# AnnaLew/pangenomix

Hardware: AMD Instinct MI355X
Metric: proteins/sec clustered at 0.8 identity + pan/core iters/sec, 400-genome set (higher is better)
Workload: dtype i32

## Files before the change

pangenomix_amd/csrc/cluster.hip:

```cpp
#include <algorithm>
#include <chrono>
#include <cstdlib>
#include <cmath>
#include <type_traits>
#include <functional>
#include <condition_variable>
#include <mutex>
#include <thread>
#include <vector>

#include "cluster_layout.h"
#include "cluster_tables.h"
#include "pgx_internal.h"

namespace {

using namespace pgxc;

constexpr uint32_t kWindowMax = 65536;
constexpr int kDiscoveryRounds = 2;
constexpr uint32_t kBlockCap = 4096;
constexpr uint32_t kBlockCapMin = 64;

constexpr uint32_t kMaxLen = 1u << 22;
// ... 1084 lines not shown
        FT_LAP(ft, 9);
    }
    flush_pairs();
#ifdef PGX_FTIME
    FT_LAP(ft, 10);
    if (lane == 0 && NEWONLY && !A.qlist) {
        for (int i = 0; i < 12; ++i) atomicAdd(&g_ftime[i], ft.acc[i]);
        atomicAdd(&g_ftime[12], 1ull);
    }
#endif
    if (lane == 0 && wave_visits) atomicAdd(&s_visits, wave_visits);
    __syncthreads();
    if (threadIdx.x == 0 && s_visits) atomicAdd(A.visits, s_visits);
}

__global__ __launch_bounds__(256) void index_strike_kernel(DevSeqs S, const uint32_t *__restrict__ list, uint32_t n,
                                                          IndexLine *__restrict__ lines, uint32_t *__restrict__ pool) {
    const uint32_t lane = threadIdx.x & 63u, rmask = entry_rmask(S);
    for (uint32_t w = blockIdx.x * 4 + (threadIdx.x >> 6); w < n; w += gridDim.x * 4) {
        const uint32_t k = list[w];
        const uint64_t o = S.off[k];
        const uint32_t nw = S.wcnt[k];
        for (uint32_t i = lane; i < nw; i += 64) {
            IndexLine &L = lines[S.wcode[o + i]];
            const uint32_t hi = L.len;
            for (uint32_t j = line_len_prev(L); j < hi; ++j) {
                uint32_t *e = j < kInline ? &L.e[j] : &pool[L.ovf + 1u + (j - kInline)];
                if ((*e & rmask) == k) { *e = rmask; break; }
            }
        }
    }
}

enum { C_NW = 0, C_NK = 1, C_EVAL0 = 2, C_BLK = 3, C_OPEN = 4, C_NEW = 5, C_SEG0 = 6, C_TOUCH = 7, C_ERR = 8, C_ROUND_OPEN = 9, C_ZERO = 10, C_WIDE = 11, C_ROUND_OPEN2 = 12, C_COUNT = 16 };
constexpr int kSelThreads = 1024;
__global__ __launch_bounds__(kSelThreads) void select_block_kernel(const unsigned long long *__restrict__ best,
                                                                  uint8_t *__restrict__ done,
                                                                  uint8_t *__restrict__ inblk, uint32_t b0,
                                                                  uint32_t nb, uint32_t block_cap,
                                                                  uint32_t *__restrict__ blk_list,
                                                                  uint32_t *__restrict__ counters,
                                                                  uint32_t *__restrict__ n_k,
                                                                  uint8_t *__restrict__ hascand_accepted,
                                                                  uint32_t window_cap, uint32_t *__restrict__ base_counters) {
    constexpr uint32_t kTiles = kWindowMax / kSelThreads;
    __shared__ uint32_t s_pre[kTiles][16];
    __shared__ uint32_t s_tile[kTiles + 1];
    const uint32_t tid = threadIdx.x, lane = tid & 63u, wave = tid >> 6;
    for (uint32_t i = tid; i < 2 * window_cap / 8; i += kSelThreads) reinterpret_cast<unsigned long long *>(hascand_accepted)[i] = 0ull;
    if (tid == 0) { *n_k = 0u; base_counters[C_TOUCH] = 0u; base_counters[C_EVAL0] = base_counters[C_NW]; }
    const uint32_t n_tiles = (nb + kSelThreads - 1) / kSelThreads;
    unsigned long long open = 0ull;
#pragma unroll 8
    for (uint32_t j = 0; j < n_tiles; ++j) {
        const uint32_t q = j * kSelThreads + tid;
        if (q >= nb) continue;
        const uint8_t ib = inblk[q];
        uint8_t d = done[q];
        const unsigned long long b = best[q];
        if (ib) { done[q] = 1; inblk[q] = 0; d = 1; }
        if (!d && b == kNoBest) open |= 1ull << j;
    }
    for (uint32_t j = 0; j < n_tiles; ++j) {
        const unsigned long long bal = __ballot((open >> j) & 1ull);
        if (lane == 0) s_pre[j][wave] = (uint32_t)__popcll(bal);
    }
    __syncthreads();
    {
        const uint32_t j = tid >> 4, w = tid & 15u;
        const uint32_t c = j < n_tiles ? s_pre[j][w] : 0u;
        uint32_t incl = c;
        for (int dd = 1; dd < 16; dd <<= 1) { const uint32_t y = __shfl_up(incl, dd, 16); if ((int)w >= dd) incl += y; }
        __syncthreads();
        if (j < n_tiles) s_pre[j][w] = incl - c;
        if (w == 15u) s_tile[j] = incl;
    }
    __syncthreads();
    if (wave == 0) {
        const uint32_t c = lane < n_tiles ? s_tile[lane] : 0u;
        uint32_t incl = c;
        for (int dd = 1; dd < 64; dd <<= 1) { const uint32_t y = __shfl_up(incl, dd); if ((int)lane >= dd) incl += y; }
        s_tile[lane] = incl - c;
        if (lane == 63u) { s_tile[kTiles] = incl; counters[0] = incl < block_cap ? incl : block_cap; counters[1] = incl; }
    }
    __syncthreads();
    for (uint32_t j = 0; j < n_tiles; ++j) {
        const bool is_open = (open >> j) & 1ull;
        const unsigned long long bal = __ballot(is_open);
        if (!is_open) continue;
        const uint32_t rank = s_tile[j] + s_pre[j][wave] + (uint32_t)__popcll(bal & ((1ull << lane) - 1ull));
        if (rank < block_cap) { const uint32_t q = j * kSelThreads + tid; blk_list[rank] = b0 + q; inblk[q] = 1; }
    }
}

__global__ __launch_bounds__(256) void list_open_kernel(const unsigned long long *__restrict__ best,
                                                       const uint8_t *__restrict__ done, uint32_t b0, uint32_t nb,
                                                       uint32_t *__restrict__ ulist, uint32_t *__restrict__ c,
                                                       uint32_t which) {
    const uint32_t q = blockIdx.x * blockDim.x + threadIdx.x;
    if (q == 0) {
        c[C_EVAL0] = c[C_NW]; c[C_SEG0] = c[C_NEW]; c[C_TOUCH] = 0u;
        c[which ? C_ROUND_OPEN : C_ROUND_OPEN2] = 0u;
    }
    if (q >= nb) return;
    if (!done[q] && best[q] == kNoBest) ulist[atomicAdd(&c[which ? C_ROUND_OPEN2 : C_ROUND_OPEN], 1u)] = b0 + q;
}
constexpr uint32_t kMaxChunks = 32;
struct Chunks { uint32_t n; uint32_t begin[kMaxChunks + 1]; };
__device__ __forceinline__ uint32_t chunk_of(const Chunks &C, uint32_t ql) {
    uint32_t c = 0;
    for (uint32_t t = 1; t < C.n; ++t) c += ql >= C.begin[t];
    return c;
}
__global__ __launch_bounds__(256) void first_open_kernel(DevSeqs S, const uint32_t *__restrict__ ulist,
                                                        const uint32_t *__restrict__ n_open, uint32_t b0,
                                                        uint32_t epoch, uint32_t *__restrict__ first, uint32_t stride,
                                                        Chunks C, const int32_t *__restrict__ req_aan,
                                                        uint8_t *__restrict__ decided) {
    const uint32_t lane = threadIdx.x & 63u, n = *n_open;
    for (uint32_t w = blockIdx.x * 4 + (threadIdx.x >> 6); w < n; w += gridDim.x * 4) {
        const uint32_t k = ulist[w], ql = k - b0, c = chunk_of(C, ql);
        const uint64_t o = S.off[k];
        const uint32_t nw = S.wcnt[k], tag = (epoch << 16) | (65535u - ql);
        uint32_t sum = 0;
        for (uint32_t i = lane; i < nw; i += 64) {
            uint32_t *slot = first + (size_t)S.wcode[o + i] * stride + c;
            const uint32_t v = *slot;
            if (v < tag) atomicMax(slot, tag);
            else if (v > tag && (v >> 16) == epoch) sum += S.wmult[o + i];
        }
        for (int d = 32; d > 0; d >>= 1) sum += __shfl_xor(sum, d);
        if (lane == 0) decided[ql] = sum != 0u && (int32_t)sum >= req_aan[k];
    }
}
__global__ __launch_bounds__(256) void certain_kernel(DevSeqs S, const uint32_t *__restrict__ ulist,
                                                     const uint32_t *__restrict__ n_open, uint32_t b0,
                                                     uint32_t both, uint32_t epoch,
                                                     const uint32_t *__restrict__ first, uint32_t stride, Chunks C,
                                                     const int32_t *__restrict__ req_aan,
                                                     const uint8_t *__restrict__ decided,
                                                     uint8_t *__restrict__ done, uint32_t *__restrict__ list,
                                                     uint32_t *__restrict__ n_list) {
    __shared__ uint32_t s_cnt[4][kMaxChunks];
    const uint32_t lane = threadIdx.x & 63u, n = *n_open;
    uint32_t *cnt = s_cnt[threadIdx.x >> 6];
    for (uint32_t w = blockIdx.x * 4 + (threadIdx.x >> 6); w < n; w += gridDim.x * 4) {
        const uint32_t k = ulist[w], ql = k - b0;
        if (decided[ql]) continue;
        const uint32_t c = chunk_of(C, ql);
        const int32_t t0 = req_aan[k];
        bool cand = false;
        for (uint32_t strand = 0; strand < (both ? 2u : 1u) && !cand; ++strand) {
            const uint32_t ks = strand ? S.n_fwd + k : k;
            const uint64_t o = S.off[ks];
            const uint32_t nw = S.wcnt[ks];
            if (lane < kMaxChunks) cnt[lane] = 0u;
            __builtin_amdgcn_fence(__ATOMIC_RELEASE, "workgroup");
            __builtin_amdgcn_wave_barrier();
            uint32_t sum = 0;
            for (uint32_t i = lane; i < nw; i += 64) {
                const uint32_t m = S.wmult[o + i];
                const uint32_t *rec = first + (size_t)S.wcode[o + i] * stride;
                for (uint32_t t4 = 0; t4 <= c; t4 += 4) {
                    uint32_t v[4];
                    if (stride >= 4) { const uint4 x = *reinterpret_cast<const uint4 *>(rec + t4); v[0] = x.x; v[1] = x.y; v[2] = x.z; v[3] = x.w; }
                    else { v[0] = rec[0]; v[1] = stride > 1 ? rec[1] : 0u; v[2] = 0u; v[3] = 0u; }
#pragma unroll
                    for (uint32_t j = 0; j < 4; ++j) {
                        const uint32_t t = t4 + j;
                        if (t > c || (v[j] >> 16) != epoch) continue;
                        if (t < c) atomicAdd(&cnt[t], m);
                        else if (65535u - (v[j] & 65535u) < ql) sum += m;
                    }
                }
            }
            for (int d = 32; d > 0; d >>= 1) sum += __shfl_xor(sum, d);
            __builtin_amdgcn_fence(__ATOMIC_RELEASE, "workgroup");
            __builtin_amdgcn_wave_barrier();
            __builtin_amdgcn_fence(__ATOMIC_ACQUIRE, "workgroup");
            uint32_t mx = lane < c ? cnt[lane] : 0u;
            mx = mx > sum ? mx : sum;
            for (int d = 32; d > 0; d >>= 1) { const uint32_t v = __shfl_xor(mx, d); mx = v > mx ? v : mx; }
            cand = mx != 0u && (int32_t)mx >= t0;
            __builtin_amdgcn_wave_barrier();
        }
        if (!cand && lane == 0) {
            done[ql] = 1;
            list[atomicAdd(n_list, 1u)] = k;
        }
    }
}

__global__ __launch_bounds__(256) void thresholds_kernel(const uint32_t *__restrict__ len, uint32_t n,
                                                        const int32_t *__restrict__ tab, uint32_t n_len,
                                                        int32_t *__restrict__ aa1, int32_t *__restrict__ aas,
                                                        int32_t *__restrict__ aan) {
    const uint32_t k = blockIdx.x * blockDim.x + threadIdx.x;
    if (k >= n) return;
    const uint32_t L = len[k];
    aa1[k] = tab[L]; aas[k] = tab[n_len + L]; aan[k] = tab[2 * n_len + L];
}


__global__ void retire_block_kernel(uint8_t *__restrict__ done, uint8_t *__restrict__ inblk, uint32_t nb, uint32_t final_,
                                    uint32_t *__restrict__ begin) {
    const uint32_t q = blockIdx.x * blockDim.x + threadIdx.x;
    if (q == 0 && begin) { begin[C_TOUCH] = 0u; begin[C_NK] = 0u; begin[C_EVAL0] = begin[C_NW]; }
    if (q < nb && inblk[q]) { done[q] = (uint8_t)final_; inblk[q] = 0; }
}
__global__ __launch_bounds__(256) void window_init_kernel(uint32_t *__restrict__ counters,
                                                         unsigned long long *__restrict__ best,
                                                         unsigned long long *__restrict__ rc_visits,
                                                         uint8_t *__restrict__ flags, uint32_t window_cap) {
    const uint32_t q = blockIdx.x * blockDim.x + threadIdx.x;
    if (q < C_COUNT && q != C_ERR) counters[q] = 0u;
    if (q >= window_cap) return;
    best[q] = kNoBest;
    if (rc_visits) rc_visits[q] = 0ull;
    if (q < 4 * window_cap / 8) reinterpret_cast<unsigned long long *>(flags)[q] = 0ull;
// ... 843 lines not shown
            if (out_strand) out_strand[i] = 0;
        }
    });
    if (n_in == 0) { if (stats) *stats = S; return PGX_OK; }

    DevBuf d_res, d_off, d_len, d_wcode, d_wmult, d_wcnt, d_aa1, d_aas, d_aan, d_lines, d_pool[2], d_idx,
        d_newbits, d_touched, d_first, d_best_own, d_rcvis, d_counters, d_visits, d_pairsW, d_pairsK, d_blk_list,
        d_ulist, d_new_list, d_flags, d_gscratch, d_order, d_list, d_gather, d_pk, d_pkoff,
        d_counters2, d_best2, d_flags2, d_pairsW2, d_gscratch2,
        d_thr, d_hugewords, d_xsend, d_xrecv,
        d_hist, d_sortcnt, d_tilesum, d_runs;
    {
        DevBuf *all[] = {&d_res, &d_off, &d_len, &d_wcode, &d_wmult, &d_wcnt, &d_aa1, &d_aas, &d_aan, &d_lines,
                         &d_pool[0], &d_pool[1], &d_idx, &d_newbits, &d_touched, &d_first, &d_best_own, &d_rcvis,
                         &d_counters, &d_visits, &d_pairsW, &d_pairsK, &d_blk_list, &d_ulist, &d_new_list, &d_flags,
                         &d_gscratch, &d_order, &d_list, &d_gather, &d_pk, &d_pkoff,
                         &d_counters2, &d_best2, &d_flags2, &d_pairsW2, &d_gscratch2, &d_thr, &d_hugewords,
                         &d_xsend, &d_xrecv, &d_hist, &d_sortcnt, &d_tilesum, &d_runs};
        int sl = 1;
        for (DevBuf *b : all) { b->ctx = ctx; b->slot = sl++; }
    }
    uint32_t n_codes = 1;
    for (int t = 0; t < P->word_len; ++t) n_codes *= nt ? 4u : (uint32_t)kNAA1;
    static_assert(kSegs == 4, "eight codes per word of the round's map");
    const uint32_t bm_words = (n_codes / 8 + 2 + 3) & ~3u;
    const bool overlap = !nt && !std::getenv("PGX_NO_OVERLAP");
    DevBuf d_in_len;
    d_in_len.ctx = ctx; d_in_len.slot = 0;
    PGX_HIP(d_in_len.alloc((size_t)n_in * 4));
    constexpr uint32_t kHistWords = H_BINS + kDevSortMaxLen + 1;
    PGX_HIP(d_hist.alloc((size_t)kHistWords * 4));
    PGX_HIP(d_idx.alloc(16));
    PGX_HIP(d_newbits.alloc(2 * (size_t)bm_words * 4 + 16));
    PGX_HIP(d_counters.alloc(C_COUNT * 4));
    PGX_HIP(d_visits.alloc(8));
    if (overlap) PGX_HIP(d_counters2.alloc(C_COUNT * 4));
    {
        ClearArgs ca{};
        auto seg = [&](DevBuf &b, size_t words) { ca.p[ca.n] = b.as<uint32_t>(); ca.words[ca.n] = (uint32_t)words; ++ca.n; };
        seg(d_hist, kHistWords);
        seg(d_newbits, 2 * (size_t)bm_words);
        seg(d_counters, C_COUNT);
        seg(d_visits, 2);
        if (overlap) seg(d_counters2, C_COUNT);
        ca.one = d_idx.as<uint32_t>();
        clear_kernel<<<1024, 256, 0, st>>>(ca);
        LAUNCH_CHECK();
    }
    {
        ProfScope prof(ctx, "seq_len_kernel", st);
        seq_len_kernel<<<(n_in + 3) / 4, 256, 0, st>>>(d_residues, d_offsets, n_in, total_in, d_in_len.as<uint32_t>());
        len_hist_kernel<<<std::min(64u, (n_in + 1023u) / 1024u), 1024, 0, st>>>(d_in_len.as<uint32_t>(), n_in, P->min_length,
                                                                               d_hist.as<uint32_t>());
    }
    LAUNCH_CHECK();
    HostVec<uint32_t> h_hist(ctx, 6, kHistWords);
    PGX_REQUIRE(h_hist.ok(), "out of host memory");
    PGX_HIP(hipMemcpyAsync(h_hist.data(), d_hist.p, (size_t)(H_BINS + kHistLds) * 4, hipMemcpyDeviceToHost, st));
    PGX_HIP(hipStreamSynchronize(st));
    const bool dev_sort = h_hist[H_OVER] == 0 && !std::getenv("PGX_HOST_PROLOGUE");
    uint32_t max_len = h_hist[H_MAX];
    if (dev_sort && max_len >= kHistLds) {
        PGX_HIP(hipMemcpyAsync(h_hist.data() + H_BINS + kHistLds, d_hist.as<uint32_t>() + H_BINS + kHistLds,
                               (size_t)(max_len + 1 - kHistLds) * 4, hipMemcpyDeviceToHost, st));
        PGX_HIP(hipStreamSynchronize(st));
    }
    phase("  seq_len + histogram + copy");
    const uint32_t *len_hist = h_hist.data() + H_BINS;
    uint32_t n = 0;
// ... 109 lines not shown
        uint64_t in_chunk = 0;
        uint32_t q = 0;
        for (; b0 + q < limit && q < window_cap; ++q) {
            const uint64_t w = h_len[b0 + q];
            if (chunking && in_chunk && in_chunk + w > chunk_words) {
                if (C.n == kMaxChunks) break;
                C.begin[C.n++] = q;
                in_chunk = 0;
            }
            in_chunk += w;
        }
        C.begin[C.n] = q;
        return q;
    };
    const bool need_gscratch = (uint64_t)max_len * 2 > kDiagLdsSmall;
    const uint32_t packed_len = nt ? kPackedLenNt : kPackedLenAa;
    const uint32_t gs_cells = (max_len + 64u) & ~63u;
    const uint32_t gs_stride = (max_len > packed_len ? 5u : 3u) * gs_cells;
    const uint32_t diag_grid = (uint32_t)std::max<uint64_t>(64, std::min<uint64_t>(8192, (4ull << 30) / ((uint64_t)gs_stride * 4)));
    const uint32_t align_grid = 1024;

    PGX_HIP(d_res.alloc(total + 16));
    PGX_HIP(d_off.alloc(((size_t)nv + 1) * 8));
    PGX_HIP(d_len.alloc((size_t)nv * 4));
    PGX_HIP(d_wcode.alloc((total + 16) * 4));
    PGX_HIP(d_wmult.alloc((total + 16) * 2));
    PGX_HIP(d_wcnt.alloc((size_t)nv * 4));
    PGX_HIP(d_pk.alloc(((size_t)total_pk + 16) * 4));
    PGX_HIP(d_pkoff.alloc(((size_t)nv + 1) * 4));
    PGX_HIP(d_aa1.alloc((size_t)n * 4));
    PGX_HIP(d_aas.alloc((size_t)n * 4));
    PGX_HIP(d_aan.alloc((size_t)n * 4));
    PGX_HIP(d_lines.alloc((size_t)n_codes * sizeof(IndexLine)));
    PGX_HIP(hipMemsetAsync(d_lines.p, 0, (size_t)n_codes * sizeof(IndexLine), st));
    PGX_HIP(d_best_own.alloc((size_t)window_cap * 8));
    PGX_HIP(d_rcvis.alloc((size_t)window_cap * 8));
    PGX_HIP(d_blk_list.alloc((size_t)kBlockCap * 4));
    PGX_HIP(d_ulist.alloc((size_t)window_cap * 4));
    PGX_HIP(d_new_list.alloc((size_t)window_cap * 4));
    PGX_HIP(d_flags.alloc(4 * (size_t)window_cap));
    PGX_HIP(d_list.alloc((size_t)pair_cap_k * 4));
    PGX_HIP(d_gather.alloc((size_t)pair_cap_k * sizeof(Pair)));
    PGX_HIP(d_pairsW.alloc((size_t)pair_cap * sizeof(Pair)));
    PGX_HIP(d_pairsK.alloc((size_t)pair_cap_k * sizeof(Pair)));
    if (need_gscratch) PGX_HIP(d_gscratch.alloc((size_t)diag_grid * gs_stride * 4));
    if (overlap) {
        if (!exchanging) PGX_HIP(d_best2.alloc((size_t)window_cap * 8));
        PGX_HIP(d_flags2.alloc(4 * (size_t)window_cap));
        PGX_HIP(d_pairsW2.alloc((size_t)pair_cap * sizeof(Pair)));
        if (need_gscratch) PGX_HIP(d_gscratch2.alloc((size_t)diag_grid * gs_stride * 4));
    }
    int pool_cur = 0;
    uint64_t pool_cap = 0;
    auto ensure_pool = [&](uint64_t entries, hipStream_t on) -> int {
        const uint64_t need = 8 * entries + 4096;
        if (need <= pool_cap) return PGX_OK;
        if (need > 0xFFFFFFF0ull) { pgx_set_error("pgx_cluster_greedy: word index too large for 32-bit pool offsets"); return PGX_ERR_CAPACITY; }
        const uint64_t want = std::min<uint64_t>(0xFFFFFFF0ull, need + need / 2);
        DevBuf &nb_ = d_pool[pool_cur ^ 1];
        PGX_HIP(nb_.alloc(want * 4));
        if (pool_cap) PGX_HIP(hipMemcpyAsync(nb_.p, d_pool[pool_cur].p, pool_cap * 4, hipMemcpyDeviceToDevice, on));
        pool_cur ^= 1;
        pool_cap = want;
        return PGX_OK;
    };
    PGX_HIP(d_order.alloc((size_t)n * 4));
    if (dev_sort) {
        uint32_t per = kSortShare;
        while ((uint64_t)((n_in + per - 1) / per) * n_runs > kSortCells) per *= 2;
        const uint32_t n_shares = (n_in + per - 1) / per, cells = n_shares * n_runs, tiles = (cells + kScanTile - 1) / kScanTile;
        PGX_HIP(d_sortcnt.alloc((size_t)cells * 4));
        PGX_HIP(d_tilesum.alloc((size_t)tiles * 4));
        uint32_t *const cnt = d_sortcnt.as<uint32_t>(), *const in_len = d_in_len.as<uint32_t>();
        ProfScope prof(ctx, "length_sort_kernels", st);
        ClearArgs ca{};
        ca.p[0] = cnt; ca.words[0] = cells; ca.n = 1;
        clear_kernel<<<std::min(2048u, (cells + 255u) / 256u), 256, 0, st>>>(ca);
        sort_count_kernel<<<(n_in + 255) / 256, 256, 0, st>>>(in_len, n_in, P->min_length, max_len, per, n_shares, cnt);
        tile_sum_kernel<<<tiles, 256, 0, st>>>(cnt, cells, d_tilesum.as<uint32_t>());
        tile_scan_kernel<<<tiles, 256, 0, st>>>(cnt, cells, d_tilesum.as<uint32_t>());
        sort_place_kernel<<<(n_shares + 3) / 4, 256, 0, st>>>(in_len, n_in, P->min_length, max_len, per, n_shares, cnt, n,
                                                              d_order.as<uint32_t>());
        LAUNCH_CHECK();
        PGX_HIP(hipMemcpyAsync(order.data(), d_order.p, (size_t)n * 4, hipMemcpyDeviceToHost, st));
    } else {
        PGX_HIP(hipMemcpyAsync(d_order.p, order.data(), (size_t)n * 4, hipMemcpyHostToDevice, st));
    }
    {
        const size_t runs_bytes = 2 * ((size_t)n_runs + 1) * 8;
        PGX_HIP(d_runs.alloc(runs_bytes));
        PGX_HIP(hipMemcpyAsync(d_runs.p, h_runs.data(), runs_bytes, hipMemcpyHostToDevice, st));
        const uint64_t *const dr_off = d_runs.as<uint64_t>();
        const uint32_t *const dr_pos = reinterpret_cast<const uint32_t *>(dr_off + n_runs + 1), *const dr_pk = dr_pos + n_runs + 1;
        layout_kernel<<<nv / 256 + 1, 256, 0, st>>>(dr_off, dr_pos, dr_pk, n_runs, max_len, n, nv, d_len.as<uint32_t>(),
                                                    d_off.as<uint64_t>(), d_pkoff.as<uint32_t>());
        LAUNCH_CHECK();
    }
    {
        ProfScope prof(ctx, "encode_gather_kernel", st);
        encode_gather_kernel<<<(n + 3) / 4, 256, 0, st>>>(d_residues, d_offsets, d_order.as<uint32_t>(),
                                                          d_off.as<uint64_t>(), d_res.as<uint8_t>(), n, nt ? 1 : 0);
        if (both)
            revcomp_kernel<<<(n + 3) / 4, 256, 0, st>>>(d_res.as<uint8_t>(), d_off.as<uint64_t>(),
                                                        d_len.as<uint32_t>(), n);
        pack5_kernel<<<(nv + 3) / 4, 256, 0, st>>>(d_res.as<uint8_t>(), d_off.as<uint64_t>(), d_len.as<uint32_t>(),
                                                   d_pkoff.as<uint32_t>(), nv, d_pk.as<uint32_t>());
    }
    LAUNCH_CHECK();
    {
        PGX_HIP(d_thr.alloc(3 * ((size_t)max_len + 1) * 4));
        PGX_HIP(hipMemcpyAsync(d_thr.p, h_thr.data(), 3 * ((size_t)max_len + 1) * 4, hipMemcpyHostToDevice, st));
        thresholds_kernel<<<(n + 255) / 256, 256, 0, st>>>(d_len.as<uint32_t>(), n, d_thr.as<int32_t>(), max_len + 1,
                                                          d_aa1.as<int32_t>(), d_aas.as<int32_t>(), d_aan.as<int32_t>());
        LAUNCH_CHECK();
    }
    phase("alloc + sort + layout + encode (enq)");
    {
// ... 9 lines not shown
            const uint32_t o = half * n;
            if (k32) {
                uint32_t slots = 65536;
                while (slots < 2u * max_len) slots *= 2;
                const uint32_t per_launch = std::min(k32, std::max(1u, (uint32_t)((256ull << 20) / ((uint64_t)slots * 8))));
                PGX_HIP(d_hugewords.alloc((size_t)per_launch * slots * 8));
                ProfScope prof(ctx, "words_kernel", st);
                for (uint32_t a = 0; a < k32; a += per_launch)
                    words_huge_kernel<<<std::min(per_launch, k32 - a), 1024, 0, st>>>(r8, o64, l32, o + a, o + std::min(k32, a + per_launch), wl, base,
                                                                                       nt, d_hugewords.as<uint32_t>(), slots, wc, wm, wn,
                                                                                       d_counters.as<uint32_t>() + C_ERR);
                LAUNCH_CHECK();
            }
            if ((rc = launch_words<32768, 1024>(ctx, st, r8, o64, l32, o + k32, o + k8, wl, base, nt, wc, wm, wn))) return rc;
            if ((rc = launch_words<8192, 1024>(ctx, st, r8, o64, l32, o + k8, o + k2, wl, base, nt, wc, wm, wn))) return rc;
            if ((rc = launch_words_hash<2048, 256>(ctx, st, r8, o64, l32, o + k2, o + k1k, wl, base, nt, wc, wm, wn))) return rc;
            if (k5 > k1k) {
                ProfScope prof(ctx, "words_kernel", st);
                words_wave_kernel<2048><<<(k5 - k1k + 3) / 4, 256, 0, st>>>(r8, o64, l32, o + k1k, o + k5, wl, base, nt, wc, wm, wn);
                LAUNCH_CHECK();
            }
            if (n > k5) {
                ProfScope prof(ctx, "words_kernel", st);
                words_wave_kernel<1024><<<(n - k5 + 3) / 4, 256, 0, st>>>(r8, o64, l32, o + k5, o + n, wl, base, nt, wc, wm, wn);
                LAUNCH_CHECK();
            }
        }
    }
    DevSeqs DS{d_res.as<uint8_t>(), d_off.as<uint64_t>(), d_len.as<uint32_t>(),
               d_wcode.as<uint32_t>(), d_wmult.as<uint16_t>(), d_wcnt.as<uint32_t>(),
               d_pk.as<uint32_t>(), d_pkoff.as<uint32_t>(), n, nt ? 4 : kNAA1, nt ? 4 : 2, nt ? 1 : 0, mshift};
    HostVec<uint32_t> h_wcnt(ctx, 8, n);
    PGX_REQUIRE(h_wcnt.ok(), "out of host memory");
    PGX_HIP(hipMemcpyAsync(h_wcnt.data(), d_wcnt.p, (size_t)n * 4, hipMemcpyDeviceToHost, st));

    phase("word lists (enqueue)");
    fill_host_layout();
    phase("host lengths + offsets");
    uint64_t max_window_words = 0;
    uint32_t max_chunks = 1;
    {
        Chunks C;
        size_t nf = 0;
        for (uint32_t b0 = 0, nbw; b0 < n; b0 += nbw) {
            while (nf < flush_at.size() && flush_at[nf] <= b0) ++nf;
            nbw = form_window(b0, C, nf < flush_at.size() ? flush_at[nf] : n);
            max_window_words = std::max<uint64_t>(max_window_words, h_off[b0 + nbw] - h_off[b0]);
            max_chunks = std::max(max_chunks, C.n);
        }
        if (!flush_at.empty())
            max_window_words = std::max<uint64_t>(max_window_words, h_off[std::min(n, window_cap)]);
    }
    if (chunking && flush_at.empty())
        max_window_words = std::max<uint64_t>(max_window_words,
            std::min<uint64_t>(h_off[std::min(n, window_cap)], (uint64_t)kMaxChunks * std::max<uint64_t>(chunk_words, max_len)));
    PGX_REQUIRE(max_window_words < 0xFFFFFFF0ull, "window too large");
    PGX_HIP(d_touched.alloc((max_window_words + 16) * sizeof(Deferred)));
    if (chunking && n > window_cap / 2) max_chunks = kMaxChunks;
    uint32_t tag_stride = 1;
    while (tag_stride < max_chunks) tag_stride *= 2;
    PGX_HIP(d_first.alloc((size_t)tag_stride * n_codes * 4 + 16));
    std::vector<uint32_t> rep_seq;
    HostVec<int32_t> cluster_of(ctx, 9, n, -1);
    HostVec<int32_t> iden_of(ctx, 10, n, -1);
    PGX_REQUIRE(cluster_of.ok() && iden_of.ok(), "out of host memory");
    Pinned<Pair> hW, hK;
    Pinned<unsigned long long> h_best, h_rcvis;
// ... 41 lines not shown
    uint8_t *const d_flags_set[2] = {d_flags.as<uint8_t>(), d_flags2.as<uint8_t>()};
    std::vector<uint8_t> status(window_cap);
    HostVec<uint8_t> strand_of(ctx, 11, n, (uint8_t)0);
    PGX_REQUIRE(strand_of.ok(), "out of host memory");
    std::vector<unsigned long long> winner_key(window_cap);
    std::vector<uint32_t> new_reps, order_k, rank_of(window_cap), bucket_k(kBlockCap + 2), fill_k(kBlockCap + 2), flight;
    auto real = [&](uint32_t k) { return k >= n ? k - n : k; };
    auto pair_key = [&](const Pair &pp) {
        return ((unsigned long long)(pp.q >= n) << 63) | ((unsigned long long)pp.minc << 32) | pp.r;
    };
    uint64_t n_rounds = 0;

    uint64_t gpu_pairs = 0, gpu_aligned = 0, gpu_aligned_bytes = 0, filter_walk_words = 0;
    auto account = [&](const Pair *pp, uint32_t cnt) {
        for (uint32_t i = 0; i < cnt; ++i) {
            ++gpu_pairs;
            if ((pp[i].flags & (F_DIAG_PASS | F_BAND_OK)) != (F_DIAG_PASS | F_BAND_OK)) continue;
            ++gpu_aligned;
            gpu_aligned_bytes += h_len[pp[i].q] + h_len[pp[i].r];
        }
    };
    auto window_error = [&](uint32_t e, uint32_t at) {
        pgx_set_error("pgx_cluster_greedy: capacity failure in the window at %u%s:%s%s%s%s%s%s", at,
                      exchanging ? " (on this or another process)" : "",
                      e & E_TOUCHED ? " append scratch list full;" : "", e & E_POOL ? " overflow pool of the word index full;" : "",
                      e & E_TABLE ? " exact table of the filter overflowed;" : "",
                      e & E_BAND ? " alignment band wider than 64 diagonals;" : "", e & E_PAIRS ? " candidate pair buffer overflow;" : "",
                      e & E_WORDMULT ? " a word occurs more than 65535 times in one sequence;" : "");
    };
    const bool trace = std::getenv("PGX_TRACE") != nullptr;
    const uint32_t filter_grid = 4096u;
    uint32_t epoch_idx = 0;
    uint32_t epoch_tag = 0;
    PGX_HIP(hipMemsetAsync(d_first.p, 0, (size_t)tag_stride * n_codes * 4, st));
    phase("window set-up");
    const auto t_loop0 = std::chrono::steady_clock::now();
    double t_resolve = 0.0, t_close = 0.0;
    uint64_t n_blocks = 0;
    g_wait_s = 0.0;
    std::function<int()> deferred;
    std::vector<uint32_t> members;
    uint64_t pending_words = 0;
    Chunks chunks;
    Pinned<uint8_t> h_taken;
    h_taken.bind(ctx, 14);
    if (!flush_at.empty()) { PGX_HIP(h_taken.reserve(n)); std::fill(h_taken.p, h_taken.p + n, (uint8_t)0); }
    auto drain = [&]() -> int {
        if (deferred) { int rc = deferred(); deferred = nullptr; if (rc) return rc; }
        PGX_HIP(hipStreamSynchronize(st_main));
        PGX_HIP(hipStreamSynchronize(ctx->stream2));
        return PGX_OK;
    };
    size_t next_flush = 0;
    bool sweeping = false;
    uint32_t sweep_at = 0;
    for (uint32_t cursor = 0, nb = 0; cursor < n;) {
        if (!sweeping && next_flush < flush_at.size() && cursor == flush_at[next_flush]) {
            ++next_flush;
            sweeping = true; sweep_at = cursor;
            int rc = drain(); if (rc) return rc;
        }
        const bool sweep = sweeping;
        const uint32_t b0 = sweep ? sweep_at : cursor;
        nb = form_window(b0, chunks, sweep || next_flush >= flush_at.size() ? n : flush_at[next_flush]);
        const int set = overlap ? (int)(S.sweeps & 1u) : 0;
        const hipStream_t st = set ? ctx->stream2 : st_main;
        uint32_t *const dc = dc_set[set];
// ... 130 lines not shown
                                                     dc + C_TOUCH, (uint32_t)max_window_words, dc + C_ERR);
            index_grow_kernel<<<256, 256, 0, st>>>(d_lines.as<IndexLine>(), d_poolp, d_idx.as<uint32_t>(),
                                                   (uint32_t)pool_cap, d_touched.as<Deferred>(), dc + C_TOUCH,
                                                   (uint32_t)max_window_words, dc + C_ERR);
            index_place_kernel<<<256, 256, 0, st>>>(d_lines.as<IndexLine>(), d_poolp, d_touched.as<Deferred>(),
                                                    dc + C_TOUCH, (uint32_t)max_window_words, reinterpret_cast<uint4 *>(next_map),
                                                    bm_words / 4);
            LAUNCH_CHECK();
            return PGX_OK;
        };
        auto filter_new_and_evaluate = [&](const uint32_t *d_lo, const uint32_t *d_hi) -> int {
            FilterArgs F = FA;
            F.epoch = epoch_idx; F.d_round_lo = d_lo; F.d_round_hi = d_hi;
            F.newbits = d_newbits.as<uint32_t>() + (size_t)(epoch_idx & 1u) * bm_words;
            {
                ProfScope prof(ctx, "filter_kernel<new>", st);
                auto kern = nt ? filter_kernel<true, true> : filter_kernel<false, true>;
                kern<<<std::min(filter_grid, (ns + 3) / 4), 256, 0, st>>>(DS, F);
            }
            LAUNCH_CHECK();
            filter_walk_words += window_words * (both ? 2 : 1) / shard_count;
            return evaluate_round();
        };
        uint32_t n_listed = 0;
        if (sweep) { int rc = begin_host_side(); if (rc) return rc; }
        if (!sweep) {
        if (overlap && S.sweeps > 1)
            PGX_HIP(hipStreamWaitEvent(st, ev.post[set ^ 1], 0));
        static const int n_disc = std::getenv("PGX_ROUNDS") ? std::atoi(std::getenv("PGX_ROUNDS")) : kDiscoveryRounds;
        for (int round = 0; round < n_disc; ++round) {
            if (++epoch_tag == 0xFFFFu) { PGX_HIP(hipMemsetAsync(d_first.p, 0, (size_t)tag_stride * n_codes * 4, st)); epoch_tag = 1; }
            const uint32_t which = (uint32_t)round & 1u;
            uint32_t *const d_n_open = dc + (which ? C_ROUND_OPEN2 : C_ROUND_OPEN);
            list_open_kernel<<<(nb + 255) / 256, 256, 0, st>>>(d_best, d_done, b0, nb, d_ulist.as<uint32_t>(), dc, which);
            LAUNCH_CHECK();
            {
                ProfScope prof(ctx, "discover_kernels", st);
                first_open_kernel<<<std::min(2048u, (nb + 3) / 4), 256, 0, st>>>(DS, d_ulist.as<uint32_t>(), d_n_open, b0,
                                                                                 epoch_tag, d_first.as<uint32_t>(), tag_stride,
                                                                                 chunks, d_aan.as<int32_t>(), d_accepted);
                certain_kernel<<<std::min(2048u, (nb + 3) / 4), 256, 0, st>>>(DS, d_ulist.as<uint32_t>(), d_n_open, b0,
                                                                              both ? 1u : 0u, epoch_tag, d_first.as<uint32_t>(), tag_stride,
                                                                              chunks,
                                                                              d_aan.as<int32_t>(), d_accepted, d_done, d_new_list.as<uint32_t>(),
                                                                              dc + C_NEW);
            }
            LAUNCH_CHECK();
            int rc = index_append(d_new_list.as<uint32_t>(), dc + C_SEG0, dc + C_NEW);
            if (rc) return rc;
            rc = filter_new_and_evaluate(dc + C_SEG0, dc + C_NEW);
            if (rc) return rc;
        }
        bool first_block = true;
        n_listed = 0;
        uint32_t n_struck = 0;
        for (;;) {
            select_block_kernel<<<1, kSelThreads, 0, st>>>(d_best, d_done, d_inblk, b0, nb, block_cap,
                                                           d_blk_list.as<uint32_t>(), dc + C_BLK, dc + C_NK,
                                                           d_hascand, window_cap, dc);
            LAUNCH_CHECK();
            {
                int rc = index_append(d_blk_list.as<uint32_t>(), dc + C_ZERO, dc + C_BLK);
                if (rc) return rc;
                FilterArgs F = FA;
                F.epoch = epoch_idx; F.d_round_lo = dc + C_ZERO; F.d_round_hi = dc + C_BLK;
                F.newbits = d_newbits.as<uint32_t>() + (size_t)(epoch_idx & 1u) * bm_words;
                F.qlist = d_blk_list.as<uint32_t>(); F.d_nq = dc + C_BLK; F.mark = d_hascand; F.count_visits = 0u;
                F.pairs = d_pairsK.as<Pair>(); F.n_pairs = dc + C_NK; F.pair_cap = pair_cap_k;
                F.shard_count = 1; F.shard_index = 0;
                ProfScope prof(ctx, "filter_kernel<block>", st);
                auto kern = nt ? filter_kernel<true, true> : filter_kernel<false, true>;
                kern<<<std::min(filter_grid, (block_cap * (both ? 2u : 1u) + 3) / 4), 256, 0, st>>>(DS, F);
            }
            LAUNCH_CHECK();
            {
                const PairSel selK{nullptr, dc + C_NK, pair_cap_k, nullptr, 0, nullptr, d_hascand, d_accepted, b0, 0, 2048};
                int rc = evaluate(d_pairsK.as<Pair>(), selK, nullptr, 0);
                if (rc) return rc;
                const PairSel selK2{nullptr, dc + C_NK, pair_cap_k, nullptr, 0, d_hascand, d_accepted, nullptr, b0, 1, 0};
                rc = evaluate(d_pairsK.as<Pair>(), selK2, nullptr, 0);
                if (rc) return rc;
            }
            {
                PubArgs pa{};
                pa.seg[0] = {dc, h_cnt.p, nullptr, C_COUNT, 1, C_COUNT};
                pa.seg[1] = {d_blk_list.as<uint32_t>(), h_blk.p, dc + C_BLK, 0, 1, block_cap};
                pa.seg[2] = {d_pairsK.as<uint32_t>(), reinterpret_cast<uint32_t *>(hK.p), dc + C_NK, 0, kPairWords, pair_cap_k};
                pa.n = 3;
                if (first_block) pa.seg[pa.n++] = {d_new_list.as<uint32_t>(), h_new.p, dc + C_NEW, 0, 1, window_cap};
                publish_kernel<<<64, 256, 0, st>>>(pa);
                LAUNCH_CHECK();
            }
// ... 155 lines not shown
            if (overlap) PGX_HIP(hipEventRecord(ev.post[set], st));
        }
        auto closed = [&, b0, st, pairsW, ev_post = ev.post[set], p_cnt = &h_ccnt_w, p_hW = &hW_w](uint32_t &nW) -> int {
            if (overlap) {
                const auto t0 = std::chrono::steady_clock::now();
                hipError_t e;
                while ((e = hipEventQuery(ev_post)) == hipErrorNotReady) {
                }
                g_wait_s += std::chrono::duration<double>(std::chrono::steady_clock::now() - t0).count();
                PGX_HIP(e);
            } else {
                PGX_HIP(spin_sync(st));
            }
            nW = p_cnt->p[C_NW];
            if (p_cnt->p[C_ERR]) { window_error(p_cnt->p[C_ERR], b0); return PGX_ERR_CAPACITY; }
            if (nW > pair_cap) {
                pgx_set_error("pgx_cluster_greedy: candidate pair buffer overflow (%u > %u) in the window at %u", nW, pair_cap, b0);
                return PGX_ERR_CAPACITY;
            }
            if (nW > p_hW->cap) {
                PGX_HIP(p_hW->reserve(nW));
                PGX_HIP(hipMemcpyAsync(p_hW->p, pairsW, (size_t)nW * sizeof(Pair), hipMemcpyDeviceToHost, st));
                PGX_HIP(spin_sync(st));
            }
            return PGX_OK;
        };
        uint32_t nW = 0;
        if (!overlap) { int rc = closed(nW); if (rc) return rc; }
        const auto t_c0 = std::chrono::steady_clock::now();
        {
            pending_words = window_words;
            deferred = [&, b0, nb, nW, sweep, closed, p_best = &h_best_w, p_hW = &hW_w]() mutable -> int {
                if (overlap) { int rc = closed(nW); if (rc) return rc; }
                const Pair *pW = p_hW->p;
                pending_words = 0;
                for (uint32_t q = 0; q < nb; ++q) {
                    if (status[q] != ST_OPEN) continue;
                    const unsigned long long key = p_best->p[q];
                    if (key == kNoBest) {
                        if (sweep) { status[q] = ST_NONE; continue; }
                        pgx_set_error("pgx_cluster_greedy: unresolved member after the last block"); return PGX_ERR_INTERNAL;
                    }
                    status[q] = ST_MEMBER;
                    winner_key[q] = key;
                    strand_of[b0 + q] = (uint8_t)(key >> 63);
                    if (sweep) h_taken.p[b0 + q] = 1;
                }
                if (both)
                    for (uint32_t q = 0; q < nb; ++q)
                        if (status[q] == ST_REP || status[q] == ST_NONE || (status[q] == ST_MEMBER && (winner_key[q] >> 63))) visits_rc += h_rcvis.p[q];
                for (uint32_t q = 0; q < nb; ++q)
                    if (status[q] == ST_REP) {
                        cluster_of[b0 + q] = (int32_t)rep_seq.size();
                        rep_seq.push_back(b0 + q);
                        S.sum_len_reps += h_len[b0 + q];
                        S.rep_words += h_wcnt[b0 + q];
                    }
                for (uint32_t q = 0; q < nb; ++q)
                    if (status[q] == ST_MEMBER) cluster_of[b0 + q] = cluster_of[(uint32_t)winner_key[q] & 0x7FFFFFFFu];
                account(pW, nW);
                bool fits = true;
                for (uint32_t i = 0; i < nW; ++i) {
                    const Pair &p = pW[i];
                    const uint32_t k = real(p.q), q = k - b0;
                    if ((p.flags & F_TOO_BIG) && (p.flags & F_DIAG_PASS)) { fits = false; continue; }
                    const unsigned long long key = pair_key(p);
// ... 107 lines not shown
```

Baseline: 16.64 million.

## Split block selection into multi-block count/place kernels and overlap setup copies

```diff
diff --git a/pangenomix_amd/csrc/cluster.hip b/pangenomix_amd/csrc/cluster.hip
--- a/pangenomix_amd/csrc/cluster.hip
+++ b/pangenomix_amd/csrc/cluster.hip
@@ -1142,63 +1142,68 @@
 
 enum { C_NW = 0, C_NK = 1, C_EVAL0 = 2, C_BLK = 3, C_OPEN = 4, C_NEW = 5, C_SEG0 = 6, C_TOUCH = 7, C_ERR = 8, C_ROUND_OPEN = 9, C_ZERO = 10, C_WIDE = 11, C_ROUND_OPEN2 = 12, C_COUNT = 16 };
 constexpr int kSelThreads = 1024;
-__global__ __launch_bounds__(kSelThreads) void select_block_kernel(const unsigned long long *__restrict__ best,
+constexpr uint32_t kSelTiles = kWindowMax / kSelThreads;
+static_assert(kSelTiles == 64, "select_place_kernel scans the tile counts with one wave");
+__global__ __launch_bounds__(kSelThreads) void select_count_kernel(const unsigned long long *__restrict__ best,
                                                                   uint8_t *__restrict__ done,
-                                                                  uint8_t *__restrict__ inblk, uint32_t b0,
-                                                                  uint32_t nb, uint32_t block_cap,
-                                                                  uint32_t *__restrict__ blk_list,
-                                                                  uint32_t *__restrict__ counters,
+                                                                  uint8_t *__restrict__ inblk, uint32_t nb,
+                                                                  uint32_t *__restrict__ tile_cnt,
                                                                   uint32_t *__restrict__ n_k,
                                                                   uint8_t *__restrict__ hascand_accepted,
                                                                   uint32_t window_cap, uint32_t *__restrict__ base_counters) {
-    constexpr uint32_t kTiles = kWindowMax / kSelThreads;
-    __shared__ uint32_t s_pre[kTiles][16];
-    __shared__ uint32_t s_tile[kTiles + 1];
-    const uint32_t tid = threadIdx.x, lane = tid & 63u, wave = tid >> 6;
-    for (uint32_t i = tid; i < 2 * window_cap / 8; i += kSelThreads) reinterpret_cast<unsigned long long *>(hascand_accepted)[i] = 0ull;
-    if (tid == 0) { *n_k = 0u; base_counters[C_TOUCH] = 0u; base_counters[C_EVAL0] = base_counters[C_NW]; }
-    const uint32_t n_tiles = (nb + kSelThreads - 1) / kSelThreads;
-    unsigned long long open = 0ull;
-#pragma unroll 8
-    for (uint32_t j = 0; j < n_tiles; ++j) {
-        const uint32_t q = j * kSelThreads + tid;
-        if (q >= nb) continue;
+    __shared__ uint32_t s_cnt;
+    const uint32_t tid = threadIdx.x, lane = tid & 63u;
+    const uint32_t q = blockIdx.x * kSelThreads + tid;
+    bool open = false;
+    if (q < nb) {
         const uint8_t ib = inblk[q];
         uint8_t d = done[q];
         const unsigned long long b = best[q];
         if (ib) { done[q] = 1; inblk[q] = 0; d = 1; }
-        if (!d && b == kNoBest) open |= 1ull << j;
-    }
-    for (uint32_t j = 0; j < n_tiles; ++j) {
-        const unsigned long long bal = __ballot((open >> j) & 1ull);
-        if (lane == 0) s_pre[j][wave] = (uint32_t)__popcll(bal);
-    }
+        open = !d && b == kNoBest;
+    }
+    for (uint32_t i = q; i < 2 * window_cap / 8; i += gridDim.x * kSelThreads) reinterpret_cast<unsigned long long *>(hascand_accepted)[i] = 0ull;
+    if (q == 0) { *n_k = 0u; base_counters[C_TOUCH] = 0u; base_counters[C_EVAL0] = base_counters[C_NW]; }
+    if (tid == 0) s_cnt = 0u;
     __syncthreads();
-    {
-        const uint32_t j = tid >> 4, w = tid & 15u;
-        const uint32_t c = j < n_tiles ? s_pre[j][w] : 0u;
-        uint32_t incl = c;
-        for (int dd = 1; dd < 16; dd <<= 1) { const uint32_t y = __shfl_up(incl, dd, 16); if ((int)w >= dd) incl += y; }
-        __syncthreads();
-        if (j < n_tiles) s_pre[j][w] = incl - c;
-        if (w == 15u) s_tile[j] = incl;
-    }
+    const unsigned long long bal = __ballot(open);
+    if (lane == 0 && bal) atomicAdd(&s_cnt, (uint32_t)__popcll(bal));
     __syncthreads();
+    if (tid == 0) tile_cnt[blockIdx.x] = s_cnt;
+}
+__global__ __launch_bounds__(kSelThreads) void select_place_kernel(const unsigned long long *__restrict__ best,
+                                                                  const uint8_t *__restrict__ done,
+                                                                  uint8_t *__restrict__ inblk, uint32_t b0,
+                                                                  uint32_t nb, uint32_t block_cap,
+                                                                  const uint32_t *__restrict__ tile_cnt,
+                                                                  uint32_t *__restrict__ blk_list,
+                                                                  uint32_t *__restrict__ counters) {
+    __shared__ uint32_t s_wave[kSelThreads / 64];
+    __shared__ uint32_t s_base;
+    const uint32_t tid = threadIdx.x, lane = tid & 63u, wave = tid >> 6;
+    const uint32_t tile = blockIdx.x, n_tiles = gridDim.x;
+    const uint32_t q = tile * kSelThreads + tid;
+    bool open = false;
+    if (q < nb) {
+        const uint8_t d = done[q];
+        const unsigned long long b = best[q];
+        open = !d && b == kNoBest;
+    }
+    const unsigned long long bal = __ballot(open);
+    if (lane == 0) s_wave[wave] = (uint32_t)__popcll(bal);
     if (wave == 0) {
-        const uint32_t c = lane < n_tiles ? s_tile[lane] : 0u;
+        const uint32_t c = lane < n_tiles ? tile_cnt[lane] : 0u;
         uint32_t incl = c;
         for (int dd = 1; dd < 64; dd <<= 1) { const uint32_t y = __shfl_up(incl, dd); if ((int)lane >= dd) incl += y; }
-        s_tile[lane] = incl - c;
-        if (lane == 63u) { s_tile[kTiles] = incl; counters[0] = incl < block_cap ? incl : block_cap; counters[1] = incl; }
+        if (lane == tile) s_base = incl - c;
+        if (lane == 63u && tile == 0u) { counters[0] = incl < block_cap ? incl : block_cap; counters[1] = incl; }
     }
     __syncthreads();
-    for (uint32_t j = 0; j < n_tiles; ++j) {
-        const bool is_open = (open >> j) & 1ull;
-        const unsigned long long bal = __ballot(is_open);
-        if (!is_open) continue;
-        const uint32_t rank = s_tile[j] + s_pre[j][wave] + (uint32_t)__popcll(bal & ((1ull << lane) - 1ull));
-        if (rank < block_cap) { const uint32_t q = j * kSelThreads + tid; blk_list[rank] = b0 + q; inblk[q] = 1; }
-    }
+    uint32_t rank = s_base;
+    if (rank >= block_cap || !open) return;
+    for (uint32_t w = 0; w < wave; ++w) rank += s_wave[w];
+    rank += __builtin_amdgcn_mbcnt_hi((uint32_t)(bal >> 32), __builtin_amdgcn_mbcnt_lo((uint32_t)bal, 0u));
+    if (rank < block_cap) { blk_list[rank] = b0 + q; inblk[q] = 1; }
 }
 
 __global__ __launch_bounds__(256) void list_open_kernel(const unsigned long long *__restrict__ best,
@@ -2202,9 +2207,9 @@
     PGX_HIP(d_hist.alloc((size_t)kHistWords * 4));
     PGX_HIP(d_idx.alloc(16));
     PGX_HIP(d_newbits.alloc(2 * (size_t)bm_words * 4 + 16));
-    PGX_HIP(d_counters.alloc(C_COUNT * 4));
+    PGX_HIP(d_counters.alloc((C_COUNT + kSelTiles) * 4));
     PGX_HIP(d_visits.alloc(8));
-    if (overlap) PGX_HIP(d_counters2.alloc(C_COUNT * 4));
+    if (overlap) PGX_HIP(d_counters2.alloc((C_COUNT + kSelTiles) * 4));
     {
         ClearArgs ca{};
         auto seg = [&](DevBuf &b, size_t words) { ca.p[ca.n] = b.as<uint32_t>(); ca.words[ca.n] = (uint32_t)words; ++ca.n; };
@@ -2380,7 +2385,12 @@
     PGX_HIP(d_aas.alloc((size_t)n * 4));
     PGX_HIP(d_aan.alloc((size_t)n * 4));
     PGX_HIP(d_lines.alloc((size_t)n_codes * sizeof(IndexLine)));
-    PGX_HIP(hipMemsetAsync(d_lines.p, 0, (size_t)n_codes * sizeof(IndexLine), st));
+    struct SideEvents {
+        hipEvent_t cleared = nullptr, sorted = nullptr, counted = nullptr, copied = nullptr;
+        ~SideEvents() { for (hipEvent_t e : {cleared, sorted, counted, copied}) if (e) (void)hipEventDestroy(e); }
+    } side;
+    for (hipEvent_t *e : {&side.cleared, &side.sorted, &side.counted, &side.copied}) PGX_HIP(hipEventCreateWithFlags(e, hipEventDisableTiming));
+    PGX_HIP(hipMemsetAsync(d_lines.p, 0, (size_t)n_codes * sizeof(IndexLine), ctx->stream2));
     PGX_HIP(d_best_own.alloc((size_t)window_cap * 8));
     PGX_HIP(d_rcvis.alloc((size_t)window_cap * 8));
     PGX_HIP(d_blk_list.alloc((size_t)kBlockCap * 4));
@@ -2430,7 +2440,9 @@
         sort_place_kernel<<<(n_shares + 3) / 4, 256, 0, st>>>(in_len, n_in, P->min_length, max_len, per, n_shares, cnt, n,
                                                               d_order.as<uint32_t>());
         LAUNCH_CHECK();
-        PGX_HIP(hipMemcpyAsync(order.data(), d_order.p, (size_t)n * 4, hipMemcpyDeviceToHost, st));
+        PGX_HIP(hipEventRecord(side.sorted, st));
+        PGX_HIP(hipStreamWaitEvent(ctx->stream2, side.sorted, 0));
+        PGX_HIP(hipMemcpyAsync(order.data(), d_order.p, (size_t)n * 4, hipMemcpyDeviceToHost, ctx->stream2));
     } else {
         PGX_HIP(hipMemcpyAsync(d_order.p, order.data(), (size_t)n * 4, hipMemcpyHostToDevice, st));
     }
@@ -2506,7 +2518,7 @@
                d_pk.as<uint32_t>(), d_pkoff.as<uint32_t>(), n, nt ? 4 : kNAA1, nt ? 4 : 2, nt ? 1 : 0, mshift};
     HostVec<uint32_t> h_wcnt(ctx, 8, n);
     PGX_REQUIRE(h_wcnt.ok(), "out of host memory");
-    PGX_HIP(hipMemcpyAsync(h_wcnt.data(), d_wcnt.p, (size_t)n * 4, hipMemcpyDeviceToHost, st));
+    PGX_HIP(hipEventRecord(side.counted, st));
 
     phase("word lists (enqueue)");
     fill_host_layout();
@@ -2614,7 +2626,13 @@
     const uint32_t filter_grid = 4096u;
     uint32_t epoch_idx = 0;
     uint32_t epoch_tag = 0;
-    PGX_HIP(hipMemsetAsync(d_first.p, 0, (size_t)tag_stride * n_codes * 4, st));
+    PGX_HIP(hipMemsetAsync(d_first.p, 0, (size_t)tag_stride * n_codes * 4, ctx->stream2));
+    PGX_HIP(hipEventRecord(side.cleared, ctx->stream2));
+    PGX_HIP(hipStreamWaitEvent(st, side.cleared, 0));
+    PGX_HIP(hipStreamWaitEvent(ctx->stream2, side.counted, 0));
+    PGX_HIP(hipMemcpyAsync(h_wcnt.data(), d_wcnt.p, (size_t)n * 4, hipMemcpyDeviceToHost, ctx->stream2));
+    PGX_HIP(hipEventRecord(side.copied, ctx->stream2));
+    bool copies_pending = true;
     phase("window set-up");
     const auto t_loop0 = std::chrono::steady_clock::now();
     double t_resolve = 0.0, t_close = 0.0;
@@ -2834,9 +2852,13 @@
         n_listed = 0;
         uint32_t n_struck = 0;
         for (;;) {
-            select_block_kernel<<<1, kSelThreads, 0, st>>>(d_best, d_done, d_inblk, b0, nb, block_cap,
-                                                           d_blk_list.as<uint32_t>(), dc + C_BLK, dc + C_NK,
-                                                           d_hascand, window_cap, dc);
+            {
+                const uint32_t n_tiles = std::max(1u, (nb + kSelThreads - 1) / kSelThreads);
+                select_count_kernel<<<n_tiles, kSelThreads, 0, st>>>(d_best, d_done, d_inblk, nb, dc + C_COUNT, dc + C_NK,
+                                                                     d_hascand, window_cap, dc);
+                select_place_kernel<<<n_tiles, kSelThreads, 0, st>>>(d_best, d_done, d_inblk, b0, nb, block_cap, dc + C_COUNT,
+                                                                     d_blk_list.as<uint32_t>(), dc + C_BLK);
+            }
             LAUNCH_CHECK();
             {
                 int rc = index_append(d_blk_list.as<uint32_t>(), dc + C_ZERO, dc + C_BLK);
@@ -3058,6 +3080,7 @@
             pending_words = window_words;
             deferred = [&, b0, nb, nW, sweep, closed, p_best = &h_best_w, p_hW = &hW_w]() mutable -> int {
                 if (overlap) { int rc = closed(nW); if (rc) return rc; }
+                if (copies_pending) { PGX_HIP(hipEventSynchronize(side.copied)); copies_pending = false; }
                 const Pair *pW = p_hW->p;
                 pending_words = 0;
                 for (uint32_t q = 0; q < nb; ++q) {
```

Result: no change. 16.62 million (-0.1%).

## Compact undecided list and restructure discovery kernels with block-wide work and prefetch

Applied to the files above, without the earlier changes.

```diff
diff --git a/pangenomix_amd/csrc/cluster.hip b/pangenomix_amd/csrc/cluster.hip
--- a/pangenomix_amd/csrc/cluster.hip
+++ b/pangenomix_amd/csrc/cluster.hip
@@ -1140,7 +1140,7 @@
     }
 }
 
-enum { C_NW = 0, C_NK = 1, C_EVAL0 = 2, C_BLK = 3, C_OPEN = 4, C_NEW = 5, C_SEG0 = 6, C_TOUCH = 7, C_ERR = 8, C_ROUND_OPEN = 9, C_ZERO = 10, C_WIDE = 11, C_ROUND_OPEN2 = 12, C_COUNT = 16 };
+enum { C_NW = 0, C_NK = 1, C_EVAL0 = 2, C_BLK = 3, C_OPEN = 4, C_NEW = 5, C_SEG0 = 6, C_TOUCH = 7, C_ERR = 8, C_ROUND_OPEN = 9, C_ZERO = 10, C_WIDE = 11, C_ROUND_OPEN2 = 12, C_UNDECIDED = 13, C_COUNT = 16 };
 constexpr int kSelThreads = 1024;
 __global__ __launch_bounds__(kSelThreads) void select_block_kernel(const unsigned long long *__restrict__ best,
                                                                   uint8_t *__restrict__ done,
@@ -1209,6 +1209,7 @@
     if (q == 0) {
         c[C_EVAL0] = c[C_NW]; c[C_SEG0] = c[C_NEW]; c[C_TOUCH] = 0u;
         c[which ? C_ROUND_OPEN : C_ROUND_OPEN2] = 0u;
+        c[C_UNDECIDED] = 0u;
     }
     if (q >= nb) return;
     if (!done[q] && best[q] == kNoBest) ulist[atomicAdd(&c[which ? C_ROUND_OPEN2 : C_ROUND_OPEN], 1u)] = b0 + q;
@@ -1224,75 +1225,113 @@
                                                         const uint32_t *__restrict__ n_open, uint32_t b0,
                                                         uint32_t epoch, uint32_t *__restrict__ first, uint32_t stride,
                                                         Chunks C, const int32_t *__restrict__ req_aan,
-                                                        uint8_t *__restrict__ decided) {
-    const uint32_t lane = threadIdx.x & 63u, n = *n_open;
-    for (uint32_t w = blockIdx.x * 4 + (threadIdx.x >> 6); w < n; w += gridDim.x * 4) {
+                                                        uint32_t *__restrict__ undecided,
+                                                        uint32_t *__restrict__ n_undecided) {
+    __shared__ uint32_t s_sum[2][4];
+    const uint32_t lane = threadIdx.x & 63u, wave = threadIdx.x >> 6, n = *n_open;
+    const bool per_wave = n > 2u * gridDim.x;
+    const uint32_t first_w = per_wave ? blockIdx.x * 4 + wave : blockIdx.x, step_w = per_wave ? gridDim.x * 4 : gridDim.x;
+    const uint32_t first_i = per_wave ? lane : threadIdx.x, step_i = per_wave ? 64u : 256u;
+    uint32_t buf = 0;
+    for (uint32_t w = first_w; w < n; w += step_w) {
         const uint32_t k = ulist[w], ql = k - b0, c = chunk_of(C, ql);
         const uint64_t o = S.off[k];
         const uint32_t nw = S.wcnt[k], tag = (epoch << 16) | (65535u - ql);
-        uint32_t sum = 0;
-        for (uint32_t i = lane; i < nw; i += 64) {
-            uint32_t *slot = first + (size_t)S.wcode[o + i] * stride + c;
+        const uint32_t last = nw ? nw - 1u : 0u;
+        uint32_t sum = 0, code = S.wcode[o + (first_i < nw ? first_i : last)], m = S.wmult[o + (first_i < nw ? first_i : last)];
+        for (uint32_t i = first_i; i < nw; i += step_i) {
+            const uint64_t at = o + (i + step_i < nw ? i + step_i : last);
+            const uint32_t ncode = S.wcode[at], nm = S.wmult[at];
+            uint32_t *slot = first + (size_t)code * stride + c;
             const uint32_t v = *slot;
             if (v < tag) atomicMax(slot, tag);
-            else if (v > tag && (v >> 16) == epoch) sum += S.wmult[o + i];
+            else if (v > tag && (v >> 16) == epoch) sum += m;
+            code = ncode; m = nm;
         }
         for (int d = 32; d > 0; d >>= 1) sum += __shfl_xor(sum, d);
-        if (lane == 0) decided[ql] = sum != 0u && (int32_t)sum >= req_aan[k];
-    }
-}
-__global__ __launch_bounds__(256) void certain_kernel(DevSeqs S, const uint32_t *__restrict__ ulist,
-                                                     const uint32_t *__restrict__ n_open, uint32_t b0,
+        if (!per_wave) {
+            if (lane == 0) s_sum[buf][wave] = sum;
+            __syncthreads();
+            sum = s_sum[buf][0] + s_sum[buf][1] + s_sum[buf][2] + s_sum[buf][3];
+            buf ^= 1u;
+        }
+        if ((per_wave ? lane : threadIdx.x) == 0 && !(sum != 0u && (int32_t)sum >= req_aan[k]))
+            undecided[atomicAdd(n_undecided, 1u)] = k;
+    }
+}
+constexpr uint32_t kCertainDepth = 4;
+template <bool kWide>
+__global__ __launch_bounds__(256) void certain_kernel(DevSeqs S, const uint32_t *__restrict__ undecided,
+                                                     const uint32_t *__restrict__ n_undecided, uint32_t b0,
                                                      uint32_t both, uint32_t epoch,
                                                      const uint32_t *__restrict__ first, uint32_t stride, Chunks C,
                                                      const int32_t *__restrict__ req_aan,
-                                                     const uint8_t *__restrict__ decided,
                                                      uint8_t *__restrict__ done, uint32_t *__restrict__ list,
                                                      uint32_t *__restrict__ n_list) {
-    __shared__ uint32_t s_cnt[4][kMaxChunks];
-    const uint32_t lane = threadIdx.x & 63u, n = *n_open;
-    uint32_t *cnt = s_cnt[threadIdx.x >> 6];
-    for (uint32_t w = blockIdx.x * 4 + (threadIdx.x >> 6); w < n; w += gridDim.x * 4) {
-        const uint32_t k = ulist[w], ql = k - b0;
-        if (decided[ql]) continue;
-        const uint32_t c = chunk_of(C, ql);
+    __shared__ uint32_t s_cnt[2][4][kMaxChunks];
+    const uint32_t tid = threadIdx.x, lane = tid & 63u, wave = tid >> 6, n = *n_undecided;
+    const uint32_t L = kWide ? stride / 4 : 1u;
+    const uint32_t g = tid / L, j = tid % L, wpi = 256u / L;
+    uint32_t buf = 0;
+    for (uint32_t w = blockIdx.x; w < n; w += gridDim.x) {
+        const uint32_t k = undecided[w], ql = k - b0, c = chunk_of(C, ql);
         const int32_t t0 = req_aan[k];
+        uint32_t lim[4];
+#pragma unroll
+        for (uint32_t jj = 0; jj < 4; ++jj) { const uint32_t t = 4 * j + jj; lim[jj] = t < c ? 65536u : t == c ? ql : 0u; }
+        const bool piece = 4 * j <= c;
         bool cand = false;
         for (uint32_t strand = 0; strand < (both ? 2u : 1u) && !cand; ++strand) {
             const uint32_t ks = strand ? S.n_fwd + k : k;
             const uint64_t o = S.off[ks];
-            const uint32_t nw = S.wcnt[ks];
-            if (lane < kMaxChunks) cnt[lane] = 0u;
-            __builtin_amdgcn_fence(__ATOMIC_RELEASE, "workgroup");
-            __builtin_amdgcn_wave_barrier();
-            uint32_t sum = 0;
-            for (uint32_t i = lane; i < nw; i += 64) {
-                const uint32_t m = S.wmult[o + i];
-                const uint32_t *rec = first + (size_t)S.wcode[o + i] * stride;
-                for (uint32_t t4 = 0; t4 <= c; t4 += 4) {
-                    uint32_t v[4];
-                    if (stride >= 4) { const uint4 x = *reinterpret_cast<const uint4 *>(rec + t4); v[0] = x.x; v[1] = x.y; v[2] = x.z; v[3] = x.w; }
-                    else { v[0] = rec[0]; v[1] = stride > 1 ? rec[1] : 0u; v[2] = 0u; v[3] = 0u; }
+            const uint32_t nw = S.wcnt[ks], last = nw ? nw - 1u : 0u;
+            uint32_t acc[4] = {0u, 0u, 0u, 0u}, code[kCertainDepth], m[kCertainDepth];
+            auto load_word = [&](uint32_t i, uint32_t &cd, uint32_t &mult) {
+                const uint64_t at = o + (i < nw ? i : last);
+                const uint32_t mm = S.wmult[at];
+                cd = S.wcode[at];
+                mult = i < nw ? mm : 0u;
+            };
 #pragma unroll
-                    for (uint32_t j = 0; j < 4; ++j) {
-                        const uint32_t t = t4 + j;
-                        if (t > c || (v[j] >> 16) != epoch) continue;
-                        if (t < c) atomicAdd(&cnt[t], m);
-                        else if (65535u - (v[j] & 65535u) < ql) sum += m;
+            for (uint32_t d = 0; d < kCertainDepth; ++d) load_word(d * wpi + g, code[d], m[d]);
+            for (uint32_t base = 0; base < nw; base += kCertainDepth * wpi) {
+                uint4 x[kCertainDepth];
+                uint32_t ncode[kCertainDepth], nm[kCertainDepth];
+#pragma unroll
+                for (uint32_t d = 0; d < kCertainDepth; ++d) load_word(base + (kCertainDepth + d) * wpi + g, ncode[d], nm[d]);
+#pragma unroll
+                for (uint32_t d = 0; d < kCertainDepth; ++d) x[d] = make_uint4(0u, 0u, 0u, 0u);
+                if (piece) {
+#pragma unroll
+                    for (uint32_t d = 0; d < kCertainDepth; ++d) {
+                        const uint32_t *rec = first + (size_t)code[d] * stride;
+                        if (kWide) x[d] = *reinterpret_cast<const uint4 *>(rec + 4 * j);
+                        else { x[d].x = rec[0]; x[d].y = rec[stride - 1]; }
                     }
                 }
-            }
-            for (int d = 32; d > 0; d >>= 1) sum += __shfl_xor(sum, d);
-            __builtin_amdgcn_fence(__ATOMIC_RELEASE, "workgroup");
-            __builtin_amdgcn_wave_barrier();
-            __builtin_amdgcn_fence(__ATOMIC_ACQUIRE, "workgroup");
-            uint32_t mx = lane < c ? cnt[lane] : 0u;
-            mx = mx > sum ? mx : sum;
-            for (int d = 32; d > 0; d >>= 1) { const uint32_t v = __shfl_xor(mx, d); mx = v > mx ? v : mx; }
+#pragma unroll
+                for (uint32_t d = 0; d < kCertainDepth; ++d) {
+                    const uint32_t v[4] = {x[d].x, x[d].y, x[d].z, x[d].w};
+#pragma unroll
+                    for (uint32_t jj = 0; jj < 4; ++jj)
+                        acc[jj] += (v[jj] >> 16) == epoch && 65535u - (v[jj] & 65535u) < lim[jj] ? m[d] : 0u;
+                    code[d] = ncode[d]; m[d] = nm[d];
+                }
+            }
+#pragma unroll
+            for (uint32_t jj = 0; jj < 4; ++jj)
+                for (uint32_t d = 32; d >= L; d >>= 1) acc[jj] += __shfl_xor(acc[jj], d);
+            if (lane < kMaxChunks / 4) {
+#pragma unroll
+                for (uint32_t jj = 0; jj < 4; ++jj) s_cnt[buf][wave][4 * lane + jj] = lane < L ? acc[jj] : 0u;
+            }
+            __syncthreads();
+            uint32_t mx = lane < kMaxChunks ? s_cnt[buf][0][lane] + s_cnt[buf][1][lane] + s_cnt[buf][2][lane] + s_cnt[buf][3][lane] : 0u;
+            for (int d = 32; d > 0; d >>= 1) { const uint32_t y = __shfl_xor(mx, d); mx = y > mx ? y : mx; }
             cand = mx != 0u && (int32_t)mx >= t0;
-            __builtin_amdgcn_wave_barrier();
-        }
-        if (!cand && lane == 0) {
+            buf ^= 1u;
+        }
+        if (!cand && tid == 0) {
             done[ql] = 1;
             list[atomicAdd(n_list, 1u)] = k;
         }
@@ -2384,7 +2423,7 @@
     PGX_HIP(d_best_own.alloc((size_t)window_cap * 8));
     PGX_HIP(d_rcvis.alloc((size_t)window_cap * 8));
     PGX_HIP(d_blk_list.alloc((size_t)kBlockCap * 4));
-    PGX_HIP(d_ulist.alloc((size_t)window_cap * 4));
+    PGX_HIP(d_ulist.alloc(2 * (size_t)window_cap * 4));
     PGX_HIP(d_new_list.alloc((size_t)window_cap * 4));
     PGX_HIP(d_flags.alloc(4 * (size_t)window_cap));
     PGX_HIP(d_list.alloc((size_t)pair_cap_k * 4));
@@ -2811,18 +2850,20 @@
             if (++epoch_tag == 0xFFFFu) { PGX_HIP(hipMemsetAsync(d_first.p, 0, (size_t)tag_stride * n_codes * 4, st)); epoch_tag = 1; }
             const uint32_t which = (uint32_t)round & 1u;
             uint32_t *const d_n_open = dc + (which ? C_ROUND_OPEN2 : C_ROUND_OPEN);
+            uint32_t *const d_undecided = d_ulist.as<uint32_t>() + window_cap;
             list_open_kernel<<<(nb + 255) / 256, 256, 0, st>>>(d_best, d_done, b0, nb, d_ulist.as<uint32_t>(), dc, which);
             LAUNCH_CHECK();
             {
                 ProfScope prof(ctx, "discover_kernels", st);
                 first_open_kernel<<<std::min(2048u, (nb + 3) / 4), 256, 0, st>>>(DS, d_ulist.as<uint32_t>(), d_n_open, b0,
                                                                                  epoch_tag, d_first.as<uint32_t>(), tag_stride,
-                                                                                 chunks, d_aan.as<int32_t>(), d_accepted);
-                certain_kernel<<<std::min(2048u, (nb + 3) / 4), 256, 0, st>>>(DS, d_ulist.as<uint32_t>(), d_n_open, b0,
-                                                                              both ? 1u : 0u, epoch_tag, d_first.as<uint32_t>(), tag_stride,
-                                                                              chunks,
-                                                                              d_aan.as<int32_t>(), d_accepted, d_done, d_new_list.as<uint32_t>(),
-                                                                              dc + C_NEW);
+                                                                                 chunks, d_aan.as<int32_t>(), d_undecided,
+                                                                                 dc + C_UNDECIDED);
+                auto certain = tag_stride >= 4 ? certain_kernel<true> : certain_kernel<false>;
+                certain<<<std::min(2048u, nb), 256, 0, st>>>(DS, d_undecided, dc + C_UNDECIDED, b0,
+                                                                    both ? 1u : 0u, epoch_tag, d_first.as<uint32_t>(), tag_stride,
+                                                                    chunks, d_aan.as<int32_t>(), d_done,
+                                                                    d_new_list.as<uint32_t>(), dc + C_NEW);
             }
             LAUNCH_CHECK();
             int rc = index_append(d_new_list.as<uint32_t>(), dc + C_SEG0, dc + C_NEW);
```

After: 16.52 million before, 16.68 million after, median of 5. About the same (+1.0%).
